# cshizhe/VLN-HAMT

Hardware: AMD Instinct MI355X
Metric: panorama-steps/sec, R2R proxy pretrain (36x768 views, 80-tok instr) (higher is better)
Workload: dtype bf16; 1 GPU; R2R 6-proxy-task pretrain step (fwd+bwd+clip+AdamW, dropout 0.1), fixed ViT features, R2R-canon model 174.8M params; per_gpu_batch=64, global_batch=64, txt_len=80, hist_len=5, views=36, task_mix=mlm:sap:sar:sprel:mrc:itm=5:1:1:1:2:2, parallelism=dp1, launch=hipGraph replay, dead_code_elimination=True

## Files before the change

### include/hamt.h

```cpp
#ifndef HAMT_H
#define HAMT_H

#include <stddef.h>
#include <stdint.h>

#ifdef __cplusplus
extern "C" {
#endif

#define HAMT_ABI_VERSION 2

typedef enum { HAMT_OK = 0, HAMT_ERR_ARG = -1, HAMT_ERR_UNSUPPORTED = -2, HAMT_ERR_LAUNCH = -3 } hamt_status;
typedef enum { HAMT_F32 = 0, HAMT_BF16 = 1,
               HAMT_U8G = 2,
               HAMT_F16 = 3 } hamt_dtype;
typedef enum { HAMT_PREC_BF16 = 0, HAMT_PREC_F32 = 1 } hamt_prec;

int hamt_version(void);
int hamt_last_error(char* buf, size_t n);
int hamt_last_kernel(char* buf, size_t n);
enum { HAMT_WS_GEMM_SPLITK = 0, HAMT_WS_COLSUM = 1, HAMT_WS_SUMSQ = 2, HAMT_WS_LN_BWD = 3, HAMT_WS_WGRAD_TABLE = 4, HAMT_WS_LNRED_TABLE = 5, HAMT_WS_VIS_EMBED_BWD = 6,
       HAMT_WS_EMBED_BWD = 7 ,
       HAMT_WS_OBJ_EMBED_BWD = 8, HAMT_WS_IMAGE_PREP = 9  };
size_t hamt_workspace_bytes(int op, const int* shape, int nshape);
// ... 113 lines not shown
typedef struct {
  const float *w_ang, *b_ang, *w_pos, *b_pos;
  const float *gamma_img, *beta_img, *gamma_ang, *beta_ang, *gamma_pos, *beta_pos;
  const float *tt, *nav, *gamma_out, *beta_out;
} hamt_obj_embed_params;
typedef struct {
  float *dw_ang, *db_ang, *dw_pos, *db_pos;
  float *dgamma_img, *dbeta_img, *dgamma_ang, *dbeta_ang, *dgamma_pos, *dbeta_pos;
  float *dtt, *dnav, *dgamma_out, *dbeta_out;
} hamt_obj_embed_grads;
int hamt_obj_embed_fwd(const hamt_obj_embed_desc* d, const hamt_obj_embed_params* p, const void* x1, const float* ang, const float* pos,
                       float* y, float* stats, const uint64_t* rng, void* stream);
int hamt_obj_embed_bwd(const hamt_obj_embed_desc* d, const hamt_obj_embed_params* p, const hamt_obj_embed_grads* g, const float* dy,
                       const void* x1, const float* ang, const float* pos, const float* stats, float* dx, void* dx16, float* ws,
                       const uint64_t* rng, void* stream);

typedef struct {
  int M, H;
  float eps, p_pre, p_post;
  uint32_t call_id;
  int Mpad16;
  int io16;
} hamt_ln_desc;
#define HAMT_LN_X_BF16 1
#define HAMT_LN_Z_BF16 2
#define HAMT_LN_X_F16 4
#define HAMT_LN_Z_F16 8
int hamt_ln_fwd(const hamt_ln_desc* d, const void* x, const float* residual, const float* gamma,
                const float* beta, void* z, float* y, void* y16, float* mean, float* rstd,
                const uint64_t* rng, void* stream);
int hamt_ln_bwd(const hamt_ln_desc* d, const float* dy, const void* z, const float* mean,
                const float* rstd, const float* gamma, float* dz, float* dx, void* dx16, float* dgamma,
                float* dbeta, float* dxsum, float* ws, const uint64_t* rng, void* stream);
int hamt_ln_bwd_add(const hamt_ln_desc* d, const float* dy, const void* z, const float* mean, const float* rstd,
                    const float* gamma, const float* add, float* dz, float* dgamma, float* dbeta, float* ws,
                    void* stream);
int hamt_ln_bwd_reduce(int M, int H, const float* ws, float* dgamma, float* dbeta, float* dxsum, void* stream);
typedef struct {
  const float* ws;
  float* dgamma;
  float* dbeta;
  float* dxsum;
  int M, H;
  int atomic;
} hamt_ln_reduce_desc;
#define HAMT_LNRED_TABLE_ENTRY 48
int hamt_ln_bwd_reduce_grouped(int n, const hamt_ln_reduce_desc* descs, void* table, size_t table_bytes, void* stream);

int hamt_gather_rows(int R, int W, const float* src, int ld_src, const int64_t* idx, const float* base,
                     int ld_base, float* out, int ld_out, int col0, void* stream);
int hamt_scatter_add_rows(int R, int W, const float* src, int ld_src, int col0, const int64_t* idx,
                          float* dst, int ld_dst, void* stream);
int hamt_scatter_add_rows_ordered(int R, int W, const float* src, int ld_src, int col0, const int64_t* idx,
                                  float* dst, int ld_dst, int T, int* ws, void* stream);
int hamt_scatter_add_rows_small(int R, int W, const float* src, int ld_src, int col0, const int64_t* idx, int T, float* dst,
                                float* ws, void* stream);

int hamt_embed_sum_fwd(int B, int L, int H, const int64_t* ids, const float* word, const float* pos,
                       const float* type_row, float* z, void* stream);
int hamt_embed_sum_bwd(int B, int L, int H, int V, const int64_t* ids, const float* dz, float* dword,
                       float* dpos, float* dtype_row, float* ws, size_t ws_bytes, void* stream);

int hamt_mean_mid_fwd(int B, int S, int H, const float* x, float* y, void* stream);
int hamt_mean_mid_bwd(int B, int S, int H, const float* dy, float* dx, void* stream);
int hamt_mul_bcast_fwd(int B, int S, int H, const float* a, const float* c, int ldc_rows, float* y, void* stream);
int hamt_mul_bcast_bwd(int B, int S, int H, const float* a, const float* c, int ldc_rows, const float* dy,
// ... 179 lines not shown
```

### vln_hamt_amd/_lib.py

```python
from __future__ import annotations

import ctypes as C
import os

_HERE = os.path.dirname(os.path.abspath(__file__))
LIB_PATH = os.path.join(_HERE, "libhamt_hip.so")

HAMT_F32, HAMT_BF16, HAMT_U8G, HAMT_F16 = 0, 1, 2, 3
PREC_BF16, PREC_F32 = 0, 1
EPI_BIAS, EPI_GELU, EPI_RELU, EPI_ACCUM, EPI_MUL_DGELU, EPI_MUL_DRELU, EPI_SAVE_PRE = 1, 2, 4, 8, 16, 32, 64
EPI_GELU_GRAD, EPI_MUL_AUX, EPI_ADD_AUX, EPI_DROPOUT = 128, 256, 512, 1024
SUMSQ_SPARSE = 2
OPT_ADAMW, OPT_ADAM, OPT_RMSPROP, OPT_SGD = 0, 1, 2, 3

vp, i32, u32, f32, sz = C.c_void_p, C.c_int, C.c_uint32, C.c_float, C.c_size_t


class GemmDesc(C.Structure):
    _fields_ = [("M", i32), ("N", i32), ("K", i32), ("lda", i32), ("ldb", i32), ("ldc", i32), ("ldaux", i32),
                ("a_kmajor", i32), ("b_kmajor", i32), ("dtype_a", i32), ("dtype_b", i32), ("dtype_c", i32),
                ("dtype_aux", i32), ("prec", i32), ("epilogue", i32), ("alpha", f32), ("ka_rows", i32), ("kb_rows", i32),
                ("p_drop", f32), ("call_id", u32), ("rng", C.c_void_p)]


# ... 67 lines not shown
                ("ldx", i32), ("ldw", i32), ("accum_dw", i32), ("accum_db", i32), ("ss", vp), ("K_valid", i32),
                ("wire_scale", f32), ("dy2", vp), ("x2", vp), ("K2", i32), ("ldy2", i32), ("ldx2", i32), ("K2_valid", i32)]


SIGNATURES = {
    "hamt_version": [],
    "hamt_last_error": [C.c_char_p, sz],
    "hamt_last_kernel": [C.c_char_p, sz],
    "hamt_workspace_bytes": [i32, C.POINTER(i32), i32],
    "hamt_gemm": [C.POINTER(GemmDesc), vp, vp, vp, vp, vp, vp],
    "hamt_gemm_ksplit": [C.POINTER(GemmDesc)],
    "hamt_gemm_ws": [C.POINTER(GemmDesc), vp, vp, vp, vp, vp, vp, sz, vp],
    "hamt_gemm_plan": [C.POINTER(GemmDesc), sz, C.c_char_p, sz],
    "hamt_cast_pad_bf16": [i32, i32, i32, i32, vp, i32, vp, i32, vp],
    "hamt_cast_pad_bf16_dropout": [i32, i32, i32, vp, i32, vp, i32, f32, u32, vp, vp],
    "hamt_cast_transpose": [i32, i32, vp, i32, i32, vp, i32, i32, vp],
    "hamt_wgrad_grouped": [i32, C.POINTER(WgradDesc), vp, sz, vp],
    "hamt_wgrad_grouped_ex": [i32, C.POINTER(WgradDesc), vp, sz, i32, vp],
    "hamt_smallk_wgrad": [i32, i32, i32, vp, i32, vp, i32, vp, i32, vp, vp],
    "hamt_colsum": [i32, i32, vp, i32, i32, vp, i32, vp, vp],
    "hamt_attn_small_fwd": [C.POINTER(AttnDesc), vp, vp, vp, vp, vp, vp, vp, vp],
    "hamt_attn_small_bwd": [C.POINTER(AttnDesc), vp, vp, vp, vp, vp, vp, vp, vp, vp, vp, vp, vp, vp],
    "hamt_attn_cls_fwd": [C.POINTER(AttnDesc), vp, vp, vp, vp, vp],
    "hamt_attn_varlen_fwd": [C.POINTER(AttnDesc), vp, vp, vp, vp, vp, vp, vp, vp],
    "hamt_attn_varlen_bwd": [C.POINTER(AttnDesc), vp, vp, vp, vp, vp, vp, vp, vp, vp, vp, vp, vp],
    "hamt_attn_varlen_cross_fwd": [C.POINTER(AttnDesc), vp, vp, vp, vp, vp, C.c_int, vp, vp, vp, vp, vp, vp],
    "hamt_attn_varlen_cross_bwd": [C.POINTER(AttnDesc), vp, vp, vp, vp, vp, C.c_int, vp, vp, vp, vp, vp, vp, vp, vp, vp, vp],
    "hamt_vis_embed_fwd": [C.POINTER(VisEmbedDesc)] + [vp] * 12,
    "hamt_vis_embed_bwd": [C.POINTER(VisEmbedDesc)] + [vp] * 18,
    "hamt_obj_embed_fwd": [C.POINTER(ObjEmbedDesc), C.POINTER(ObjEmbedParams)] + [vp] * 7,
    "hamt_obj_embed_bwd": [C.POINTER(ObjEmbedDesc), C.POINTER(ObjEmbedParams), C.POINTER(ObjEmbedGrads)] + [vp] * 10,
    "hamt_ln_fwd": [C.POINTER(LnDesc), vp, vp, vp, vp, vp, vp, vp, vp, vp, vp, vp],
    "hamt_ln_bwd": [C.POINTER(LnDesc), vp, vp, vp, vp, vp, vp, vp, vp, vp, vp, vp, vp, vp, vp],
    "hamt_ln_bwd_add": [C.POINTER(LnDesc), vp, vp, vp, vp, vp, vp, vp, vp, vp, vp, vp],
    "hamt_ln_bwd_reduce": [i32, i32, vp, vp, vp, vp, vp],
    "hamt_ln_bwd_reduce_grouped": [i32, vp, vp, sz, vp],
    "hamt_gather_rows": [i32, i32, vp, i32, vp, vp, i32, vp, i32, i32, vp],
    "hamt_scatter_add_rows": [i32, i32, vp, i32, i32, vp, vp, i32, vp],
    "hamt_scatter_add_rows_small": [i32, i32, vp, i32, i32, vp, i32, vp, vp, vp],
    "hamt_scatter_add_rows_ordered": [i32, i32, vp, i32, i32, vp, vp, i32, i32, vp, vp],
    "hamt_embed_sum_fwd": [i32, i32, i32, vp, vp, vp, vp, vp, vp],
    "hamt_embed_sum_bwd": [i32, i32, i32, i32, vp, vp, vp, vp, vp, vp, sz, vp],
    "hamt_mean_mid_fwd": [i32, i32, i32, vp, vp, vp],
    "hamt_mean_mid_bwd": [i32, i32, i32, vp, vp, vp],
    "hamt_mul_bcast_fwd": [i32, i32, i32, vp, vp, i32, vp, vp],
    "hamt_mul_bcast_bwd": [i32, i32, i32, vp, vp, i32, vp, vp, vp, vp],
    "hamt_sum_rows": [i32, i32, i32, vp, i32, vp, vp, vp],
    "hamt_patchify": [i32, i32, i32, i32, i32, vp, vp, i32, i32, i32, vp],
    "hamt_image_prep": [C.POINTER(ImagePrepDesc), vp, vp, vp, vp, vp, vp, sz, vp],
    "hamt_image_resample_taps": [i32, i32, i32, i32, i32, vp, vp, vp, i32],
    "hamt_image_resample": [C.POINTER(ImageResampleDesc), vp, vp, vp, vp, vp, vp, vp],
    "hamt_add3": [sz, vp, vp, vp, vp, vp],
    "hamt_dropout": [sz, vp, vp, f32, u32, vp, vp],
    "hamt_cast_f32_bf16": [sz, vp, vp, vp],
    "hamt_unpack_padded": [vp, vp, i32, i32, i32, i32, vp, vp],
    "hamt_seq_masks": [vp, i32, i32, i32, vp, vp, vp],
    "hamt_wire_pack_bf16": [C.c_size_t, vp, vp, f32, vp],
    "hamt_wire_unpack_bf16": [C.c_size_t, vp, vp, vp],
    "hamt_fill_where_zero": [sz, vp, vp, f32, vp],
    "hamt_act_bwd": [sz, vp, vp, i32, vp, vp],
    "hamt_ce_fwd": [i32, i32, vp, i32, vp, vp, vp, vp],
    "hamt_ce_bwd": [i32, i32, vp, i32, vp, vp, vp, vp, i32, vp],
    "hamt_mse_fwd": [sz, vp, vp, vp, vp],
    "hamt_mse_bwd": [sz, vp, vp, vp, vp, vp],
    "hamt_kl_fwd": [i32, i32, vp, i32, vp, i32, vp, vp, vp],
    "hamt_kl_bwd": [i32, i32, vp, i32, vp, i32, vp, vp, vp, i32, vp],
# ... 48 lines not shown
        raise HamtError(f"{LIB_PATH} is missing: build it with `python vln_hamt_amd/csrc/build.py` "
                        "(there is no CPU/PyTorch fallback for the HAMT kernels)")
    import torch
    lib = C.CDLL(LIB_PATH)
    for name, args in SIGNATURES.items():
        fn = getattr(lib, name)
        fn.argtypes = args
        fn.restype = sz if name == "hamt_workspace_bytes" else i32
    if lib.hamt_version() != 2:
        raise HamtError("libhamt_hip.so ABI version mismatch")
    _lib = lib
    return lib


def last_error() -> str:
    buf = C.create_string_buffer(512)
    load().hamt_last_error(buf, 512)
    return buf.value.decode(errors="replace")


def last_kernel() -> str:
    buf = C.create_string_buffer(160)
    load().hamt_last_kernel(buf, 160)
    return buf.value.decode(errors="replace")


def gemm_plan(desc: GemmDesc, ws_bytes=None):
    buf = C.create_string_buffer(160)
    ks = load().hamt_gemm_plan(C.byref(desc), sz(-1).value if ws_bytes is None else ws_bytes, buf, 160)
    check(min(ks, 0), "hamt_gemm_plan")
    return ks, buf.value.decode(errors="replace")


def workspace_bytes(op: int, *shape) -> int:
    arr = (i32 * max(1, len(shape)))(*shape)
    return int(load().hamt_workspace_bytes(op, arr, len(shape)))


WS_GEMM_SPLITK, WS_COLSUM, WS_SUMSQ, WS_LN_BWD, WS_WGRAD_TABLE, WS_LNRED_TABLE, WS_VIS_EMBED_BWD, WS_EMBED_BWD, WS_OBJ_EMBED_BWD = range(9)
WS_IMAGE_PREP = 9


def check(rc: int, name: str):
    if rc != 0:
        raise HamtError(f"{name} failed (status {rc}): {last_error()}")
```

### vln_hamt_amd/csrc/ln_row.h

```cpp
#pragma once
#include "common.h"

enum { LN_F32 = 0, LN_BF16 = 1, LN_F16 = 4 };
constexpr int LN_ANGLE_K = 4;

__device__ __forceinline__ float4 zero4() { return make_float4(0.f, 0.f, 0.f, 0.f); }
__device__ __forceinline__ float4 load_row4(const void* xv, size_t o, int fmt) {
  float4 a;
  if (fmt & LN_F16) {
    const uint2 u = *(const uint2*)((const bf16_t*)xv + o);
    unpack_h2(u.x, a.x, a.y); unpack_h2(u.y, a.z, a.w);
  } else if (fmt & LN_BF16) {
    const uint2 u = *(const uint2*)((const bf16_t*)xv + o);
    a = make_float4(__uint_as_float(u.x << 16), __uint_as_float(u.x & 0xffff0000u), __uint_as_float(u.y << 16), __uint_as_float(u.y & 0xffff0000u));
  } else a = *(const float4*)((const float*)xv + o);
  return a;
}
__device__ __forceinline__ void store_bf4(bf16_t* img, size_t o, const float4 r) { *(uint2*)(img + o) = make_uint2(pack_bf2(r.x, r.y), pack_bf2(r.z, r.w)); }
__device__ __forceinline__ void zero_pad_rows(bf16_t* img, int H, int first, int Mpad16, int step, int lane) {
  for (int row = first; row < Mpad16; row += step)
    for (int c = lane * 4; c < H; c += 256) *(uint2*)(img + (size_t)row * H + c) = make_uint2(0u, 0u);
}

__device__ __forceinline__ float sum4(const float4 v) { return v.x + v.y + v.z + v.w; }
__device__ __forceinline__ float dot4(const float4 a, const float4 b) { return a.x * b.x + a.y * b.y + a.z * b.z + a.w * b.w; }
__device__ __forceinline__ float4 mul4(const float4 a, const float4 b) { return make_float4(a.x * b.x, a.y * b.y, a.z * b.z, a.w * b.w); }
__device__ __forceinline__ float4 scale4(const float4 a, float s) { return make_float4(a.x * s, a.y * s, a.z * s, a.w * s); }
__device__ __forceinline__ void acc4(float4& t, const float4 a) { t.x += a.x; t.y += a.y; t.z += a.z; t.w += a.w; }
__device__ __forceinline__ void fmacc4(float4& t, const float4 a, const float4 b) { t.x += a.x * b.x; t.y += a.y * b.y; t.z += a.z * b.z; t.w += a.w * b.w; }
__device__ __forceinline__ void fmacc4(float4& t, const float4 a, float s) { t.x += a.x * s; t.y += a.y * s; t.z += a.z * s; t.w += a.w * s; }
__device__ __forceinline__ float sqdev4(const float4 v, float m) {
  const float e0 = v.x - m, e1 = v.y - m, e2 = v.z - m, e3 = v.w - m;
  return e0 * e0 + e1 * e1 + e2 * e2 + e3 * e3;
}
__device__ __forceinline__ float4 norm4(const float4 v, float m, float r) {
  return make_float4((v.x - m) * r, (v.y - m) * r, (v.z - m) * r, (v.w - m) * r);
}
__device__ __forceinline__ float4 affine4(const float4 n, const float4 g, const float4 b) {
  return make_float4(n.x * g.x + b.x, n.y * g.y + b.y, n.z * g.z + b.z, n.w * g.w + b.w);
}
__device__ __forceinline__ float4 ln_dx4(const float4 u, const float4 n, float cu, float eu, float r) {
  return make_float4(r * (u.x - cu - n.x * eu), r * (u.y - cu - n.y * eu), r * (u.z - cu - n.z * eu), r * (u.w - cu - n.w * eu));
}
__device__ __forceinline__ float4 keep4(RngKey k, int row, int c, float p, float inv_keep) {
  float f[4];
  drop_scale4(k, hamt_mix32((uint32_t)row ^ k.k0), (uint32_t)(c >> 2), p, inv_keep, f);
  return make_float4(f[0], f[1], f[2], f[3]);
}

__device__ __forceinline__ float4 angle_proj4(const float* __restrict__ W, const float* __restrict__ b, int c, const float4 x) {
  const float4* w = (const float4*)(W + (size_t)c * LN_ANGLE_K);
  const float4 w0 = w[0], w1 = w[1], w2 = w[2], w3 = w[3];
  const float4 bb = *(const float4*)(b + c);
  float4 a;
  a.x = bb.x + x.x * w0.x + x.y * w0.y + x.z * w0.z + x.w * w0.w;
  a.y = bb.y + x.x * w1.x + x.y * w1.y + x.z * w1.z + x.w * w1.w;
  a.z = bb.z + x.x * w2.x + x.y * w2.y + x.z * w2.z + x.w * w2.w;
  a.w = bb.w + x.x * w3.x + x.y * w3.y + x.z * w3.z + x.w * w3.w;
  return a;
}

template <int NV, int NWV>
__device__ __forceinline__ void block_partial(const float4 (&t)[NV], float* __restrict__ ws, size_t vec, int H) {
  __shared__ float4 red[NWV][NV * 64];
  const int lane = threadIdx.x & 63, w = threadIdx.x >> 6;
#pragma unroll
  for (int i = 0; i < NV; ++i) red[w][i * 64 + lane] = t[i];
  __syncthreads();
  for (int e = threadIdx.x; e < NV * 64; e += 64 * NWV) {
    const int c = e * 4;
    if (c < H) {
      float4 s = red[0][e];
#pragma unroll
      for (int k = 1; k < NWV; ++k) acc4(s, red[k][e]);
      *(float4*)(ws + vec * H + c) = s;
// ... 39 lines not shown
```

### vln_hamt_amd/csrc/norm.hip

```cpp
#include "ln_row.h"

namespace {

constexpr uint32_t POST_SALT = 0x5bd1e995u;

static_assert(HAMT_LN_X_BF16 == LN_BF16 && HAMT_LN_X_F16 == LN_F16 && HAMT_LN_Z_BF16 == 2 * LN_BF16 && HAMT_LN_Z_F16 == 2 * LN_F16, "io16 layout");
__device__ __forceinline__ int ln_xfmt(int io16) { return io16 & (LN_BF16 | LN_F16); }
__device__ __forceinline__ int ln_zfmt(int io16) { return (io16 >> 1) & (LN_BF16 | LN_F16); }

template <int NV>
__global__ __launch_bounds__(256) void ln_fwd_kernel(hamt_ln_desc d, const void* __restrict__ xv,
                                                     const float* __restrict__ res, const float* __restrict__ gamma,
                                                     const float* __restrict__ beta, void* __restrict__ zv,
                                                     float* __restrict__ y, bf16_t* __restrict__ y16,
                                                     float* __restrict__ mean_o, float* __restrict__ rstd_o,
                                                     const uint64_t* __restrict__ rng) {
  const int lane = threadIdx.x & 63, w = threadIdx.x >> 6;
  const int row = blockIdx.x * 4 + w;
  const int H = d.H;
  if (row >= d.M) {
    if (y16) zero_pad_rows(y16, H, row, d.Mpad16, gridDim.x * 4, lane);
    return;
  }
  const RngKey kpre = rng_key(rng, d.call_id), kpost = rng_key(rng, d.call_id ^ POST_SALT);
  const float ik_pre = d.p_pre > 0.f ? 1.0f / (1.0f - d.p_pre) : 1.0f, ik_post = d.p_post > 0.f ? 1.0f / (1.0f - d.p_post) : 1.0f;
  const int xfmt = ln_xfmt(d.io16);
  float4 v[NV];
  float sum = 0.f;
#pragma unroll
  for (int i = 0; i < NV; ++i) {
    const int c = (i * 64 + lane) * 4;
    if (c < H) {
      const size_t o = (size_t)row * H + c;
      float4 a = load_row4(xv, o, xfmt);
      if (d.p_pre > 0.f) a = mul4(a, keep4(kpre, row, c, d.p_pre, ik_pre));
      if (res) acc4(a, *(const float4*)(res + o));
      v[i] = a;
      sum += sum4(a);
    } else v[i] = zero4();
  }
  const float mean = wave_sum(sum) / (float)H;
  float sq = 0.f;
#pragma unroll
  for (int i = 0; i < NV; ++i)
    if ((i * 64 + lane) * 4 < H) sq += sqdev4(v[i], mean);
  const float rstd = rsqrtf(wave_sum(sq) / (float)H + d.eps);
#pragma unroll
  for (int i = 0; i < NV; ++i) {
    const int c = (i * 64 + lane) * 4;
    if (c < H) {
      const size_t o = (size_t)row * H + c;
      if (zv) {
        if (d.io16 & HAMT_LN_Z_F16) *(uint2*)((bf16_t*)zv + o) = make_uint2(pack_h2(v[i].x, v[i].y), pack_h2(v[i].z, v[i].w));
        else if (d.io16 & HAMT_LN_Z_BF16) store_bf4((bf16_t*)zv, o, v[i]);
        else *(float4*)((float*)zv + o) = v[i];
      }
      float4 r = affine4(norm4(v[i], mean, rstd), *(const float4*)(gamma + c), *(const float4*)(beta + c));
      if (d.p_post > 0.f) r = mul4(r, keep4(kpost, row, c, d.p_post, ik_post));
      if (y) *(float4*)(y + o) = r;
      if (y16) store_bf4(y16, o, r);
    }
  }
  if (lane == 0) { mean_o[row] = mean; rstd_o[row] = rstd; }
}

template <int NV, int NWV>
__global__ __launch_bounds__(64 * NWV) void ln_bwd_kernel(hamt_ln_desc d, const float* __restrict__ dy,
                                                     const void* __restrict__ zv, const float* __restrict__ mean_i,
                                                     const float* __restrict__ rstd_i, const float* __restrict__ gamma,
                                                     float* __restrict__ dz, float* __restrict__ dx, bf16_t* __restrict__ dx16,
                                                     float* __restrict__ ws, const uint64_t* __restrict__ rng,
                                                     const float* __restrict__ add) {
  const int lane = threadIdx.x & 63, w = threadIdx.x >> 6;
  const int H = d.H;
  if (dx16 && blockIdx.x == 0) zero_pad_rows(dx16, H, d.M + w, d.Mpad16, NWV, lane);
  const RngKey kpre = rng_key(rng, d.call_id), kpost = rng_key(rng, d.call_id ^ POST_SALT);
  const float ik_pre = d.p_pre > 0.f ? 1.0f / (1.0f - d.p_pre) : 1.0f, ik_post = d.p_post > 0.f ? 1.0f / (1.0f - d.p_post) : 1.0f;
  const int zfmt = ln_zfmt(d.io16);
  float4 gam[NV], dg[NV], db[NV], dxs[NV];
#pragma unroll
  for (int i = 0; i < NV; ++i) {
    const int c = (i * 64 + lane) * 4;
    gam[i] = c < H ? *(const float4*)(gamma + c) : zero4();
    dg[i] = zero4(); db[i] = zero4(); dxs[i] = zero4();
  }
  for (int row = blockIdx.x * NWV + w; row < d.M; row += gridDim.x * NWV) {
    const float mean = mean_i[row], rstd = rstd_i[row];
    float4 g[NV], xh[NV];
    float s1 = 0.f, s2 = 0.f;
#pragma unroll
    for (int i = 0; i < NV; ++i) {
      const int c = (i * 64 + lane) * 4;
      if (c < H) {
        const size_t o = (size_t)row * H + c;
        float4 a = *(const float4*)(dy + o);
        if (d.p_post > 0.f) a = mul4(a, keep4(kpost, row, c, d.p_post, ik_post));
        const float4 h = norm4(load_row4(zv, o, zfmt), mean, rstd);
        fmacc4(dg[i], a, h);
        acc4(db[i], a);
        a = mul4(a, gam[i]);
        s1 += a.x + a.y + a.z + a.w;
        s2 += a.x * h.x + a.y * h.y + a.z * h.z + a.w * h.w;
        g[i] = a; xh[i] = h;
      }
    }
    const float c1 = wave_sum(s1) / (float)H, c2 = wave_sum(s2) / (float)H;
#pragma unroll
    for (int i = 0; i < NV; ++i) {
      const int c = (i * 64 + lane) * 4;
      if (c < H) {
        const size_t o = (size_t)row * H + c;
        float4 r = ln_dx4(g[i], xh[i], c1, c2, rstd);
        if (add) {
          const float4 q = *(const float4*)(add + o);
          *(float4*)(dz + o) = make_float4(r.x + q.x, r.y + q.y, r.z + q.z, r.w + q.w);
        } else *(float4*)(dz + o) = r;
        if (d.p_pre > 0.f) r = mul4(r, keep4(kpre, row, c, d.p_pre, ik_pre));
        if (dx) *(float4*)(dx + o) = r;
        if (dx16) store_bf4(dx16, o, r);
        acc4(dxs[i], r);
      }
    }
  }
  __shared__ float4 red[NWV > 4 ? NWV / 2 : 4][3][NV * 64];
#pragma unroll
  for (int half = NWV / 2; half >= 4; half >>= 1) {
    if (w >= half && w < 2 * half) {
#pragma unroll
      for (int i = 0; i < NV; ++i) { red[w - half][0][i * 64 + lane] = dg[i]; red[w - half][1][i * 64 + lane] = db[i]; red[w - half][2][i * 64 + lane] = dxs[i]; }
    }
    __syncthreads();
    if (w < half) {
#pragma unroll
      for (int i = 0; i < NV; ++i) {
        const float4 a = red[w][0][i * 64 + lane], b = red[w][1][i * 64 + lane], c = red[w][2][i * 64 + lane];
        acc4(dg[i], a); acc4(db[i], b); acc4(dxs[i], c);
      }
    }
    __syncthreads();
  }
  if (w < 4) {
#pragma unroll
    for (int i = 0; i < NV; ++i) { red[w][0][i * 64 + lane] = dg[i]; red[w][1][i * 64 + lane] = db[i]; red[w][2][i * 64 + lane] = dxs[i]; }
  }
  __syncthreads();
  if (w < 3) {
#pragma unroll
    for (int i = 0; i < NV; ++i) {
      const int c = (i * 64 + lane) * 4;
      if (c < H) {
        float4 a = red[0][w][i * 64 + lane], b = red[1][w][i * 64 + lane], cc = red[2][w][i * 64 + lane], e = red[3][w][i * 64 + lane];
        *(float4*)(ws + ((size_t)blockIdx.x * 3 + w) * H + c) = make_float4(a.x + b.x + cc.x + e.x, a.y + b.y + cc.y + e.y, a.z + b.z + cc.z + e.z, a.w + b.w + cc.w + e.w);
      }
    }
  }
}

__global__ __launch_bounds__(1024) void ln_bwd_reduce_kernel(int nb, int H, const float* __restrict__ ws, float* __restrict__ dgamma,
                                                             float* __restrict__ dbeta, float* __restrict__ dxsum) {
  const int c = blockIdx.x * 64 + (threadIdx.x & 63), ph = threadIdx.x >> 6;
  const int which = c / H, col = c % H;
  float s = 0.f;
  if (c < 3 * H)
    for (int b = ph; b < nb; b += 16) s += ws[((size_t)b * 3 + which) * H + col];
  __shared__ float red[16][64];
// ... 35 lines not shown
  const int blk = blockIdx.x % bpe;
  if (blk * 64 >= 3 * q.H) return;
  int which, col;
  float4 t;
  if (!ln_reduce4(blk, q.nb, q.H, q.ws, which, col, t)) return;
  float* o = which == 0 ? q.dgamma : (which == 1 ? q.dbeta : q.dxsum);
  if (!o) return;
  if ((q.atomic >> which) & 1) {
    atomicAdd(o + col, t.x); atomicAdd(o + col + 1, t.y); atomicAdd(o + col + 2, t.z); atomicAdd(o + col + 3, t.w);
  } else *(float4*)(o + col) = t;
}

}

extern "C" int hamt_ln_fwd(const hamt_ln_desc* d, const void* x, const float* residual, const float* gamma,
                           const float* beta, void* z, float* y, void* y16, float* mean, float* rstd,
                           const uint64_t* rng, void* stream) {
  HAMT_CHECK_ARG(d && x && gamma && beta && (y || y16) && mean && rstd, "hamt_ln_fwd: null pointer");
  HAMT_CHECK_ARG(d->H % 4 == 0 && d->H >= 4 && d->H <= 1024, "hamt_ln_fwd: H=%d unsupported (need H%%4==0, H<=1024)", d->H);
  HAMT_CHECK_ARG(d->p_pre >= 0.f && d->p_pre < 1.f && d->p_post >= 0.f && d->p_post < 1.f, "hamt_ln_fwd: bad dropout p");
  HAMT_CHECK_ARG((d->io16 & (HAMT_LN_X_BF16 | HAMT_LN_X_F16)) != (HAMT_LN_X_BF16 | HAMT_LN_X_F16) && (d->io16 & (HAMT_LN_Z_BF16 | HAMT_LN_Z_F16)) != (HAMT_LN_Z_BF16 | HAMT_LN_Z_F16),
                 "hamt_ln_fwd: io16 = %d names two formats for one tensor", d->io16);
  if (d->M == 0) return HAMT_OK;
  const int rows = (y16 && d->Mpad16 > d->M) ? d->Mpad16 : d->M;
  dim3 grid((rows + 3) / 4), block(256);
  hipStream_t s = as_stream(stream);
#define LAUNCH(NV) hipLaunchKernelGGL((ln_fwd_kernel<NV>), grid, block, 0, s, *d, x, residual, gamma, beta, z, y, (bf16_t*)y16, mean, rstd, rng)
  LN_ROW_DISPATCH(d->H, LAUNCH)
#undef LAUNCH
  HAMT_CHECK_LAUNCH("hamt_ln_fwd");
  return HAMT_OK;
}

static void ln_bwd_geometry(int M, int* nwv_out, int* nb_out) {
  static const int force_w = getenv("HAMT_LN_BWD_WAVES") ? atoi(getenv("HAMT_LN_BWD_WAVES")) : 0;
  const int nwv = force_w ? force_w : (M >= 2048 ? 16 : (M >= 1024 ? 8 : 4));
  int nb = (M + nwv - 1) / nwv;
  if (nb > 256) nb = 256;
  *nwv_out = nwv;
  *nb_out = nb;
}
static void ln_bwd_reduce_launch(int nb, int H, const float* ws, float* dgamma, float* dbeta, float* dxsum, hipStream_t s) {
  const bool al = H % 64 == 0 && (((uintptr_t)dgamma | (uintptr_t)dbeta | (uintptr_t)dxsum | (uintptr_t)ws) % 16) == 0;
  if (al) hipLaunchKernelGGL(ln_bwd_reduce4_kernel, dim3(3 * H / 64), dim3(256), 0, s, nb, H, ws, dgamma, dbeta, dxsum);
  else hipLaunchKernelGGL(ln_bwd_reduce_kernel, dim3((3 * H + 63) / 64), dim3(1024), 0, s, nb, H, ws, dgamma, dbeta, dxsum);
}

static int ln_bwd_impl(const hamt_ln_desc* d, const float* dy, const void* z, const float* mean,
                       const float* rstd, const float* gamma, float* dz, float* dx, void* dx16, float* dgamma,
                       float* dbeta, float* dxsum, float* ws, const uint64_t* rng, const float* add, void* stream) {
  HAMT_CHECK_ARG(d && dy && z && mean && rstd && gamma && dz && ws, "hamt_ln_bwd: null pointer");
  HAMT_CHECK_ARG(d->H % 4 == 0 && d->H >= 4 && d->H <= 1024, "hamt_ln_bwd: H=%d unsupported", d->H);
  HAMT_CHECK_ARG(!(d->p_pre > 0.f) || dx || dx16, "hamt_ln_bwd: p_pre > 0 needs dx or dx16");
  if (d->M == 0) return HAMT_OK;
  int nwv, nb;
  ln_bwd_geometry(d->M, &nwv, &nb);
  hipStream_t s = as_stream(stream);
  float* dxx = d->p_pre > 0.f ? dx : nullptr;
#define LAUNCH2(NV, W) hipLaunchKernelGGL((ln_bwd_kernel<NV, W>), dim3(nb), dim3(64 * W), 0, s, *d, dy, z, mean, rstd, gamma, dz, dxx, (bf16_t*)dx16, ws, rng, add)
#define LAUNCH(NV) { if (nwv == 16) LAUNCH2(NV, 16); else if (nwv == 8) LAUNCH2(NV, 8); else LAUNCH2(NV, 4); }
  LN_ROW_DISPATCH(d->H, LAUNCH)
#undef LAUNCH
#undef LAUNCH2
  if (dgamma || dbeta || dxsum) ln_bwd_reduce_launch(nb, d->H, ws, dgamma, dbeta, dxsum, s);
  HAMT_CHECK_LAUNCH("hamt_ln_bwd");
  return HAMT_OK;
}

extern "C" int hamt_ln_bwd(const hamt_ln_desc* d, const float* dy, const void* z, const float* mean,
                           const float* rstd, const float* gamma, float* dz, float* dx, void* dx16, float* dgamma,
                           float* dbeta, float* dxsum, float* ws, const uint64_t* rng, void* stream) {
  return ln_bwd_impl(d, dy, z, mean, rstd, gamma, dz, dx, dx16, dgamma, dbeta, dxsum, ws, rng, nullptr, stream);
}

extern "C" int hamt_ln_bwd_add(const hamt_ln_desc* d, const float* dy, const void* z, const float* mean,
                               const float* rstd, const float* gamma, const float* add, float* dz, float* dgamma,
                               float* dbeta, float* ws, void* stream) {
  HAMT_CHECK_ARG(add && d && !(d->p_pre > 0.f) && !(d->p_post > 0.f), "hamt_ln_bwd_add: needs `add`, and no dropout inside the LayerNorm");
  return ln_bwd_impl(d, dy, z, mean, rstd, gamma, dz, nullptr, nullptr, dgamma, dbeta, nullptr, ws, nullptr, add, stream);
}

extern "C" int hamt_ln_bwd_reduce(int M, int H, const float* ws, float* dgamma, float* dbeta, float* dxsum, void* stream) {
  HAMT_CHECK_ARG(ws && M >= 0 && H % 4 == 0 && H >= 4 && H <= 1024, "hamt_ln_bwd_reduce: bad argument");
  if (M == 0 || !(dgamma || dbeta || dxsum)) return HAMT_OK;
  int nwv, nb;
  ln_bwd_geometry(M, &nwv, &nb);
  ln_bwd_reduce_launch(nb, H, ws, dgamma, dbeta, dxsum, as_stream(stream));
  HAMT_CHECK_LAUNCH("hamt_ln_bwd_reduce");
  return HAMT_OK;
}

extern "C" int hamt_ln_bwd_reduce_grouped(int n, const hamt_ln_reduce_desc* descs, void* table, size_t table_bytes, void* stream) {
  HAMT_CHECK_ARG(n >= 0 && (n == 0 || (descs && table)), "hamt_ln_bwd_reduce_grouped: bad argument");
  if (n == 0) return HAMT_OK;
  HAMT_CHECK_ARG((size_t)n * sizeof(LnRedEntry) <= table_bytes, "hamt_ln_bwd_reduce_grouped: table too small (%zu bytes needed)", (size_t)n * sizeof(LnRedEntry));
  hipStream_t s = as_stream(stream);
  LnRedEntry* tab = (LnRedEntry*)table;
  int hmax = 0;
  for (int i = 0; i < n; ++i) {
    const hamt_ln_reduce_desc& d = descs[i];
    HAMT_CHECK_ARG(d.ws && d.M > 0 && d.H % 64 == 0 && d.H <= 1024, "hamt_ln_bwd_reduce_grouped: entry %d: needs ws, M > 0, H %% 64 == 0 (H = %d)", i, d.H);
    HAMT_CHECK_ARG((((uintptr_t)d.ws | (uintptr_t)d.dgamma | (uintptr_t)d.dbeta | (uintptr_t)d.dxsum) % 16) == 0, "hamt_ln_bwd_reduce_grouped: entry %d: pointers must be 16-byte aligned", i);
    hmax = d.H > hmax ? d.H : hmax;
  }
  for (int b0 = 0; b0 < n; b0 += LNRED_CHUNK) {
    LnRedChunk ch;
    const int cnt = n - b0 < LNRED_CHUNK ? n - b0 : LNRED_CHUNK;
    for (int i = 0; i < cnt; ++i) {
      const hamt_ln_reduce_desc& d = descs[b0 + i];
      int nwv, nb;
      ln_bwd_geometry(d.M, &nwv, &nb);
      ch.e[i] = LnRedEntry{d.ws, d.dgamma, d.dbeta, d.dxsum, nb, d.H, d.atomic, 0};
    }
    hipLaunchKernelGGL(ln_red_table_write_kernel, dim3(1), dim3(64), 0, s, ch, tab, b0, cnt);
  }
  const int bpe = 3 * hmax / 64;
  hipLaunchKernelGGL(ln_bwd_reduce_grouped_kernel, dim3(n * bpe), dim3(256), 0, s, tab, bpe);
  HAMT_CHECK_LAUNCH("hamt_ln_bwd_reduce_grouped");
  return HAMT_OK;
}
```

Baseline: 6651 panorama-steps/s.

## Restructure LayerNorm backward: contiguous row chunks, shared gamma, fused dy sum entry

Reworks the LayerNorm backward kernel so each block handles a contiguous chunk of rows rather than a grid-strided set. Gamma is staged in shared memory instead of registers, loads are issued up front per row, and the z format is specialized at compile time. A new hamt_ln_bwd_sum entry sums two upstream gradients inside the kernel, and the wave count is capped for wide rows. The aim is lower register pressure and better memory-level parallelism, plus removal of a separate add pass when callers adopt the new entry. The cost is extra shared memory and a barrier, and the reduction order changes slightly.

Result: no change. 6669 panorama-steps/s, median of 6 (+0.3%).

```diff
diff --git a/include/hamt.h b/include/hamt.h
--- a/include/hamt.h
+++ b/include/hamt.h
@@ -169,6 +169,10 @@
 int hamt_ln_bwd(const hamt_ln_desc* d, const float* dy, const void* z, const float* mean,
                 const float* rstd, const float* gamma, float* dz, float* dx, void* dx16, float* dgamma,
                 float* dbeta, float* dxsum, float* ws, const uint64_t* rng, void* stream);
+int hamt_ln_bwd_sum(const hamt_ln_desc* d, const float* dy, const float* dy2, const void* z, const float* mean,
+                    const float* rstd, const float* gamma, float* dz, float* dx, void* dx16, float* dgamma,
+                    float* dbeta, float* dxsum, float* ws, const uint64_t* rng, void* stream);
+int hamt_ln_bwd_plan(int M, int H, int* waves, int* blocks, int* rows);
 int hamt_ln_bwd_add(const hamt_ln_desc* d, const float* dy, const void* z, const float* mean, const float* rstd,
                     const float* gamma, const float* add, float* dz, float* dgamma, float* dbeta, float* ws,
                     void* stream);
diff --git a/vln_hamt_amd/_lib.py b/vln_hamt_amd/_lib.py
--- a/vln_hamt_amd/_lib.py
+++ b/vln_hamt_amd/_lib.py
@@ -123,6 +123,8 @@
     "hamt_obj_embed_bwd": [C.POINTER(ObjEmbedDesc), C.POINTER(ObjEmbedParams), C.POINTER(ObjEmbedGrads)] + [vp] * 10,
     "hamt_ln_fwd": [C.POINTER(LnDesc), vp, vp, vp, vp, vp, vp, vp, vp, vp, vp, vp],
     "hamt_ln_bwd": [C.POINTER(LnDesc), vp, vp, vp, vp, vp, vp, vp, vp, vp, vp, vp, vp, vp, vp],
+    "hamt_ln_bwd_sum": [C.POINTER(LnDesc), vp, vp, vp, vp, vp, vp, vp, vp, vp, vp, vp, vp, vp, vp, vp],
+    "hamt_ln_bwd_plan": [i32, i32, C.POINTER(i32), C.POINTER(i32), C.POINTER(i32)],
     "hamt_ln_bwd_add": [C.POINTER(LnDesc), vp, vp, vp, vp, vp, vp, vp, vp, vp, vp, vp],
     "hamt_ln_bwd_reduce": [i32, i32, vp, vp, vp, vp, vp],
     "hamt_ln_bwd_reduce_grouped": [i32, vp, vp, sz, vp],
@@ -237,6 +239,12 @@
     return ks, buf.value.decode(errors="replace")
 
 
+def ln_bwd_plan(M: int, H: int):
+    w, b, r = i32(), i32(), i32()
+    check(load().hamt_ln_bwd_plan(M, H, C.byref(w), C.byref(b), C.byref(r)), "hamt_ln_bwd_plan")
+    return w.value, b.value, r.value
+
+
 def workspace_bytes(op: int, *shape) -> int:
     arr = (i32 * max(1, len(shape)))(*shape)
     return int(load().hamt_workspace_bytes(op, arr, len(shape)))
diff --git a/vln_hamt_amd/csrc/ln_bwd_plan.h b/vln_hamt_amd/csrc/ln_bwd_plan.h
--- /dev/null
+++ b/vln_hamt_amd/csrc/ln_bwd_plan.h
@@ -0,0 +1,23 @@
+#pragma once
+
+constexpr int LN_BWD_MAX_BLOCKS = 256;
+
+struct LnBwdTuning {
+  int waves;
+};
+
+struct LnBwdPlan {
+  int waves;
+  int blocks;
+  int rows;
+};
+
+static inline LnBwdPlan ln_bwd_plan(int M, int H, LnBwdTuning t = LnBwdTuning{0}) {
+  LnBwdPlan p;
+  p.waves = (t.waves == 4 || t.waves == 8 || t.waves == 16) ? t.waves : (M >= 2048 ? 16 : (M >= 1024 ? 8 : 4));
+  if (H > 768 && p.waves > 8) p.waves = 8;
+  p.rows = 1;
+  const int nb = (M + p.waves - 1) / p.waves;
+  p.blocks = nb > LN_BWD_MAX_BLOCKS ? LN_BWD_MAX_BLOCKS : (nb < 1 ? 1 : nb);
+  return p;
+}
diff --git a/vln_hamt_amd/csrc/ln_row.h b/vln_hamt_amd/csrc/ln_row.h
--- a/vln_hamt_amd/csrc/ln_row.h
+++ b/vln_hamt_amd/csrc/ln_row.h
@@ -14,6 +14,23 @@
     const uint2 u = *(const uint2*)((const bf16_t*)xv + o);
     a = make_float4(__uint_as_float(u.x << 16), __uint_as_float(u.x & 0xffff0000u), __uint_as_float(u.y << 16), __uint_as_float(u.y & 0xffff0000u));
   } else a = *(const float4*)((const float*)xv + o);
+  return a;
+}
+__device__ __forceinline__ float4 load_raw4(const void* xv, size_t o, int fmt) {
+  if (fmt & (LN_F16 | LN_BF16)) {
+    const uint2 u = *(const uint2*)((const bf16_t*)xv + o);
+    return make_float4(__uint_as_float(u.x), __uint_as_float(u.y), 0.f, 0.f);
+  }
+  return *(const float4*)((const float*)xv + o);
+}
+__device__ __forceinline__ float4 raw_row4(const float4 r, int fmt) {
+  const uint32_t ux = __float_as_uint(r.x), uy = __float_as_uint(r.y);
+  float4 a = r;
+  if (fmt & LN_F16) {
+    unpack_h2(ux, a.x, a.y); unpack_h2(uy, a.z, a.w);
+  } else if (fmt & LN_BF16) {
+    a = make_float4(__uint_as_float(ux << 16), __uint_as_float(ux & 0xffff0000u), __uint_as_float(uy << 16), __uint_as_float(uy & 0xffff0000u));
+  }
   return a;
 }
 __device__ __forceinline__ void store_bf4(bf16_t* img, size_t o, const float4 r) { *(uint2*)(img + o) = make_uint2(pack_bf2(r.x, r.y), pack_bf2(r.z, r.w)); }
@@ -41,6 +58,20 @@
 }
 __device__ __forceinline__ float4 ln_dx4(const float4 u, const float4 n, float cu, float eu, float r) {
   return make_float4(r * (u.x - cu - n.x * eu), r * (u.y - cu - n.y * eu), r * (u.z - cu - n.z * eu), r * (u.w - cu - n.w * eu));
+}
+__device__ __forceinline__ void ln_bwd_acc4(const float4 a, const float4 h, const float4 gm, float4& dg, float4& db, float4& u, float& s1, float& s2) {
+#pragma clang fp contract(off)
+  dg.x = __builtin_fmaf(a.x, h.x, dg.x); dg.y = __builtin_fmaf(a.y, h.y, dg.y); dg.z = __builtin_fmaf(a.z, h.z, dg.z); dg.w = __builtin_fmaf(a.w, h.w, dg.w);
+  db.x = a.x + db.x; db.y = a.y + db.y; db.z = a.z + db.z; db.w = a.w + db.w;
+  u = make_float4(a.x * gm.x, a.y * gm.y, a.z * gm.z, a.w * gm.w);
+  const float hy = h.y * u.y, hz = h.z * u.z, hw = h.w * u.w;
+  s1 = s1 + ((__builtin_fmaf(a.y, gm.y, u.x) + u.z) + u.w);
+  s2 = s2 + ((__builtin_fmaf(h.x, u.x, hy) + hz) + hw);
+}
+__device__ __forceinline__ float4 ln_bwd_dx4(const float4 u, const float4 n, float cu, float eu, float r) {
+#pragma clang fp contract(off)
+  return make_float4(r * __builtin_fmaf(-eu, n.x, u.x - cu), r * __builtin_fmaf(-eu, n.y, u.y - cu), r * __builtin_fmaf(-eu, n.z, u.z - cu),
+                     r * __builtin_fmaf(-eu, n.w, u.w - cu));
 }
 __device__ __forceinline__ float4 keep4(RngKey k, int row, int c, float p, float inv_keep) {
   float f[4];
diff --git a/vln_hamt_amd/csrc/norm.hip b/vln_hamt_amd/csrc/norm.hip
--- a/vln_hamt_amd/csrc/norm.hip
+++ b/vln_hamt_amd/csrc/norm.hip
@@ -1,4 +1,5 @@
 #include "ln_row.h"
+#include "ln_bwd_plan.h"
 
 namespace {
 
@@ -64,73 +65,111 @@
   if (lane == 0) { mean_o[row] = mean; rstd_o[row] = rstd; }
 }
 
+template <int NV>
+__device__ __forceinline__ bool ln_live(int i, int c, int H) { return i < NV - 1 || c < H; }
+
+template <int NV, int NWV, int ZFMT>
+__device__ __forceinline__ void ln_bwd_rows(const hamt_ln_desc& d, const int first, const int n, const int w, const int lane,
+                                            const float* __restrict__ dy, const float* __restrict__ dy2, const void* __restrict__ zv,
+                                            const float* __restrict__ mean_i, const float* __restrict__ rstd_i, float* __restrict__ dz,
+                                            float* __restrict__ dx, bf16_t* __restrict__ dx16, const float* __restrict__ add,
+                                            const RngKey kpre, const RngKey kpost, const float ik_pre, const float ik_post,
+                                            const float4* gam, float4 (&dg)[NV], float4 (&db)[NV], float4 (&dxs)[NV]) {
+  const int H = d.H;
+  for (int row = first + w; row < first + n; row += NWV) {
+    float4 g[NV], xh[NV];
+    const float mean = mean_i[row], rstd = rstd_i[row];
+#pragma unroll
+    for (int i = 0; i < NV; ++i) {
+      const int c = (i * 64 + lane) * 4;
+      g[i] = *(const float4*)(dy + (size_t)row * H + (ln_live<NV>(i, c, H) ? c : 0));
+    }
+    if (dy2) {
+      float4 q[NV];
+#pragma unroll
+      for (int i = 0; i < NV; ++i) {
+        const int c = (i * 64 + lane) * 4;
+        q[i] = *(const float4*)(dy2 + (size_t)row * H + (ln_live<NV>(i, c, H) ? c : 0));
+      }
+#pragma unroll
+      for (int i = 0; i < NV; ++i) acc4(g[i], q[i]);
+    }
+#pragma unroll
+    for (int i = 0; i < NV; ++i) {
+      const int c = (i * 64 + lane) * 4;
+      xh[i] = load_raw4(zv, (size_t)row * H + (ln_live<NV>(i, c, H) ? c : 0), ZFMT);
+    }
+    float s1 = 0.f, s2 = 0.f;
+#pragma unroll
+    for (int i = 0; i < NV; ++i) {
+      const int c = (i * 64 + lane) * 4;
+      if (ln_live<NV>(i, c, H)) {
+        float4 a = g[i];
+        if (d.p_post > 0.f) a = mul4(a, keep4(kpost, row, c, d.p_post, ik_post));
+        const float4 h = norm4(raw_row4(xh[i], ZFMT), mean, rstd);
+        ln_bwd_acc4(a, h, gam[i * 64 + lane], dg[i], db[i], g[i], s1, s2);
+        xh[i] = h;
+      }
+    }
+    const float c1 = wave_sum(s1) / (float)H, c2 = wave_sum(s2) / (float)H;
+#pragma unroll
+    for (int i = 0; i < NV; ++i) {
+      const int c = (i * 64 + lane) * 4;
+      if (ln_live<NV>(i, c, H)) {
+        const size_t o = (size_t)row * H + c;
+        float4 t = ln_bwd_dx4(g[i], xh[i], c1, c2, rstd);
+        if (add) {
+          const float4 q = *(const float4*)(add + o);
+          *(float4*)(dz + o) = make_float4(t.x + q.x, t.y + q.y, t.z + q.z, t.w + q.w);
+        } else *(float4*)(dz + o) = t;
+        if (d.p_pre > 0.f) t = mul4(t, keep4(kpre, row, c, d.p_pre, ik_pre));
+        if (dx) *(float4*)(dx + o) = t;
+        if (dx16) store_bf4(dx16, o, t);
+        acc4(dxs[i], t);
+      }
+    }
+  }
+}
+
 template <int NV, int NWV>
 __global__ __launch_bounds__(64 * NWV) void ln_bwd_kernel(hamt_ln_desc d, const float* __restrict__ dy,
                                                      const void* __restrict__ zv, const float* __restrict__ mean_i,
                                                      const float* __restrict__ rstd_i, const float* __restrict__ gamma,
                                                      float* __restrict__ dz, float* __restrict__ dx, bf16_t* __restrict__ dx16,
                                                      float* __restrict__ ws, const uint64_t* __restrict__ rng,
-                                                     const float* __restrict__ add) {
-  const int lane = threadIdx.x & 63, w = threadIdx.x >> 6;
+                                                     const float* __restrict__ add, const float* __restrict__ dy2) {
+  const int lane = threadIdx.x & 63, w = __builtin_amdgcn_readfirstlane(threadIdx.x >> 6);
   const int H = d.H;
   if (dx16 && blockIdx.x == 0) zero_pad_rows(dx16, H, d.M + w, d.Mpad16, NWV, lane);
   const RngKey kpre = rng_key(rng, d.call_id), kpost = rng_key(rng, d.call_id ^ POST_SALT);
   const float ik_pre = d.p_pre > 0.f ? 1.0f / (1.0f - d.p_pre) : 1.0f, ik_post = d.p_post > 0.f ? 1.0f / (1.0f - d.p_post) : 1.0f;
   const int zfmt = ln_zfmt(d.io16);
-  float4 gam[NV], dg[NV], db[NV], dxs[NV];
+  __shared__ float4 gam[NV * 64];
+  float4 dg[NV], db[NV], dxs[NV];
 #pragma unroll
   for (int i = 0; i < NV; ++i) {
     const int c = (i * 64 + lane) * 4;
-    gam[i] = c < H ? *(const float4*)(gamma + c) : zero4();
+    if (w == 0) gam[i * 64 + lane] = c < H ? *(const float4*)(gamma + c) : zero4();
     dg[i] = zero4(); db[i] = zero4(); dxs[i] = zero4();
   }
-  for (int row = blockIdx.x * NWV + w; row < d.M; row += gridDim.x * NWV) {
-    const float mean = mean_i[row], rstd = rstd_i[row];
-    float4 g[NV], xh[NV];
-    float s1 = 0.f, s2 = 0.f;
-#pragma unroll
-    for (int i = 0; i < NV; ++i) {
-      const int c = (i * 64 + lane) * 4;
-      if (c < H) {
-        const size_t o = (size_t)row * H + c;
-        float4 a = *(const float4*)(dy + o);
-        if (d.p_post > 0.f) a = mul4(a, keep4(kpost, row, c, d.p_post, ik_post));
-        const float4 h = norm4(load_row4(zv, o, zfmt), mean, rstd);
-        fmacc4(dg[i], a, h);
-        acc4(db[i], a);
-        a = mul4(a, gam[i]);
-        s1 += a.x + a.y + a.z + a.w;
-        s2 += a.x * h.x + a.y * h.y + a.z * h.z + a.w * h.w;
-        g[i] = a; xh[i] = h;
-      }
-    }
-    const float c1 = wave_sum(s1) / (float)H, c2 = wave_sum(s2) / (float)H;
-#pragma unroll
-    for (int i = 0; i < NV; ++i) {
-      const int c = (i * 64 + lane) * 4;
-      if (c < H) {
-        const size_t o = (size_t)row * H + c;
-        float4 r = ln_dx4(g[i], xh[i], c1, c2, rstd);
-        if (add) {
-          const float4 q = *(const float4*)(add + o);
-          *(float4*)(dz + o) = make_float4(r.x + q.x, r.y + q.y, r.z + q.z, r.w + q.w);
-        } else *(float4*)(dz + o) = r;
-        if (d.p_pre > 0.f) r = mul4(r, keep4(kpre, row, c, d.p_pre, ik_pre));
-        if (dx) *(float4*)(dx + o) = r;
-        if (dx16) store_bf4(dx16, o, r);
-        acc4(dxs[i], r);
-      }
-    }
-  }
+  __syncthreads();
+  const int q = d.M / (int)gridDim.x, rem = d.M % (int)gridDim.x, b = blockIdx.x;
+  const int first = b * q + (b < rem ? b : rem), n = q + (b < rem ? 1 : 0);
+#define LN_BWD_ROWS(F) ln_bwd_rows<NV, NWV, F>(d, first, n, w, lane, dy, dy2, zv, mean_i, rstd_i, dz, dx, dx16, add, kpre, kpost, ik_pre, ik_post, gam, dg, db, dxs)
+  if (zfmt & LN_F16) LN_BWD_ROWS(LN_F16);
+  else if (zfmt & LN_BF16) LN_BWD_ROWS(LN_BF16);
+  else LN_BWD_ROWS(LN_F32);
+#undef LN_BWD_ROWS
   __shared__ float4 red[NWV > 4 ? NWV / 2 : 4][3][NV * 64];
 #pragma unroll
-  for (int half = NWV / 2; half >= 4; half >>= 1) {
-    if (w >= half && w < 2 * half) {
+  for (int n = NWV; n > 4; n /= 2) {
+    const int half = n / 2;
+    if (w >= half && w < n) {
 #pragma unroll
       for (int i = 0; i < NV; ++i) { red[w - half][0][i * 64 + lane] = dg[i]; red[w - half][1][i * 64 + lane] = db[i]; red[w - half][2][i * 64 + lane] = dxs[i]; }
     }
     __syncthreads();
-    if (w < half) {
+    if (w < n - half) {
 #pragma unroll
       for (int i = 0; i < NV; ++i) {
         const float4 a = red[w][0][i * 64 + lane], b = red[w][1][i * 64 + lane], c = red[w][2][i * 64 + lane];
@@ -232,13 +271,20 @@
   return HAMT_OK;
 }
 
-static void ln_bwd_geometry(int M, int* nwv_out, int* nb_out) {
+static LnBwdTuning ln_bwd_tuning() {
   static const int force_w = getenv("HAMT_LN_BWD_WAVES") ? atoi(getenv("HAMT_LN_BWD_WAVES")) : 0;
-  const int nwv = force_w ? force_w : (M >= 2048 ? 16 : (M >= 1024 ? 8 : 4));
-  int nb = (M + nwv - 1) / nwv;
-  if (nb > 256) nb = 256;
-  *nwv_out = nwv;
-  *nb_out = nb;
+  return LnBwdTuning{force_w};
+}
+template <int NV>
+static void ln_bwd_launch(const LnBwdPlan& p, hipStream_t s, const hamt_ln_desc& d, const float* dy, const void* z, const float* mean, const float* rstd,
+                          const float* gamma, float* dz, float* dx, bf16_t* dx16, float* ws, const uint64_t* rng, const float* add, const float* dy2) {
+#define LAUNCH3(W) hipLaunchKernelGGL((ln_bwd_kernel<NV, W>), dim3(p.blocks), dim3(64 * W), 0, s, d, dy, z, mean, rstd, gamma, dz, dx, dx16, ws, rng, add, dy2)
+  if constexpr (NV < 4) {
+    if (p.waves == 16) { LAUNCH3(16); return; }
+  }
+  if (p.waves == 8) LAUNCH3(8);
+  else LAUNCH3(4);
+#undef LAUNCH3
 }
 static void ln_bwd_reduce_launch(int nb, int H, const float* ws, float* dgamma, float* dbeta, float* dxsum, hipStream_t s) {
   const bool al = H % 64 == 0 && (((uintptr_t)dgamma | (uintptr_t)dbeta | (uintptr_t)dxsum | (uintptr_t)ws) % 16) == 0;
@@ -246,23 +292,20 @@
   else hipLaunchKernelGGL(ln_bwd_reduce_kernel, dim3((3 * H + 63) / 64), dim3(1024), 0, s, nb, H, ws, dgamma, dbeta, dxsum);
 }
 
-static int ln_bwd_impl(const hamt_ln_desc* d, const float* dy, const void* z, const float* mean,
+static int ln_bwd_impl(const hamt_ln_desc* d, const float* dy, const float* dy2, const void* z, const float* mean,
                        const float* rstd, const float* gamma, float* dz, float* dx, void* dx16, float* dgamma,
                        float* dbeta, float* dxsum, float* ws, const uint64_t* rng, const float* add, void* stream) {
   HAMT_CHECK_ARG(d && dy && z && mean && rstd && gamma && dz && ws, "hamt_ln_bwd: null pointer");
   HAMT_CHECK_ARG(d->H % 4 == 0 && d->H >= 4 && d->H <= 1024, "hamt_ln_bwd: H=%d unsupported", d->H);
   HAMT_CHECK_ARG(!(d->p_pre > 0.f) || dx || dx16, "hamt_ln_bwd: p_pre > 0 needs dx or dx16");
   if (d->M == 0) return HAMT_OK;
-  int nwv, nb;
-  ln_bwd_geometry(d->M, &nwv, &nb);
+  const LnBwdPlan p = ln_bwd_plan(d->M, d->H, ln_bwd_tuning());
   hipStream_t s = as_stream(stream);
   float* dxx = d->p_pre > 0.f ? dx : nullptr;
-#define LAUNCH2(NV, W) hipLaunchKernelGGL((ln_bwd_kernel<NV, W>), dim3(nb), dim3(64 * W), 0, s, *d, dy, z, mean, rstd, gamma, dz, dxx, (bf16_t*)dx16, ws, rng, add)
-#define LAUNCH(NV) { if (nwv == 16) LAUNCH2(NV, 16); else if (nwv == 8) LAUNCH2(NV, 8); else LAUNCH2(NV, 4); }
+#define LAUNCH(NV) ln_bwd_launch<NV>(p, s, *d, dy, z, mean, rstd, gamma, dz, dxx, (bf16_t*)dx16, ws, rng, add, dy2)
   LN_ROW_DISPATCH(d->H, LAUNCH)
 #undef LAUNCH
-#undef LAUNCH2
-  if (dgamma || dbeta || dxsum) ln_bwd_reduce_launch(nb, d->H, ws, dgamma, dbeta, dxsum, s);
+  if (dgamma || dbeta || dxsum) ln_bwd_reduce_launch(p.blocks, d->H, ws, dgamma, dbeta, dxsum, s);
   HAMT_CHECK_LAUNCH("hamt_ln_bwd");
   return HAMT_OK;
 }
@@ -270,22 +313,35 @@
 extern "C" int hamt_ln_bwd(const hamt_ln_desc* d, const float* dy, const void* z, const float* mean,
                            const float* rstd, const float* gamma, float* dz, float* dx, void* dx16, float* dgamma,
                            float* dbeta, float* dxsum, float* ws, const uint64_t* rng, void* stream) {
-  return ln_bwd_impl(d, dy, z, mean, rstd, gamma, dz, dx, dx16, dgamma, dbeta, dxsum, ws, rng, nullptr, stream);
+  return ln_bwd_impl(d, dy, nullptr, z, mean, rstd, gamma, dz, dx, dx16, dgamma, dbeta, dxsum, ws, rng, nullptr, stream);
+}
+
+extern "C" int hamt_ln_bwd_sum(const hamt_ln_desc* d, const float* dy, const float* dy2, const void* z, const float* mean,
+                               const float* rstd, const float* gamma, float* dz, float* dx, void* dx16, float* dgamma,
+                               float* dbeta, float* dxsum, float* ws, const uint64_t* rng, void* stream) {
+  return ln_bwd_impl(d, dy, dy2, z, mean, rstd, gamma, dz, dx, dx16, dgamma, dbeta, dxsum, ws, rng, nullptr, stream);
 }
 
 extern "C" int hamt_ln_bwd_add(const hamt_ln_desc* d, const float* dy, const void* z, const float* mean,
                                const float* rstd, const float* gamma, const float* add, float* dz, float* dgamma,
                                float* dbeta, float* ws, void* stream) {
   HAMT_CHECK_ARG(add && d && !(d->p_pre > 0.f) && !(d->p_post > 0.f), "hamt_ln_bwd_add: needs `add`, and no dropout inside the LayerNorm");
-  return ln_bwd_impl(d, dy, z, mean, rstd, gamma, dz, nullptr, nullptr, dgamma, dbeta, nullptr, ws, nullptr, add, stream);
+  return ln_bwd_impl(d, dy, nullptr, z, mean, rstd, gamma, dz, nullptr, nullptr, dgamma, dbeta, nullptr, ws, nullptr, add, stream);
+}
+
+extern "C" int hamt_ln_bwd_plan(int M, int H, int* waves, int* blocks, int* rows) {
+  HAMT_CHECK_ARG(M >= 1 && H % 4 == 0 && H >= 4 && H <= 1024, "hamt_ln_bwd_plan: bad argument (M = %d, H = %d)", M, H);
+  const LnBwdPlan p = ln_bwd_plan(M, H, ln_bwd_tuning());
+  if (waves) *waves = p.waves;
+  if (blocks) *blocks = p.blocks;
+  if (rows) *rows = p.rows;
+  return HAMT_OK;
 }
 
 extern "C" int hamt_ln_bwd_reduce(int M, int H, const float* ws, float* dgamma, float* dbeta, float* dxsum, void* stream) {
   HAMT_CHECK_ARG(ws && M >= 0 && H % 4 == 0 && H >= 4 && H <= 1024, "hamt_ln_bwd_reduce: bad argument");
   if (M == 0 || !(dgamma || dbeta || dxsum)) return HAMT_OK;
-  int nwv, nb;
-  ln_bwd_geometry(M, &nwv, &nb);
-  ln_bwd_reduce_launch(nb, H, ws, dgamma, dbeta, dxsum, as_stream(stream));
+  ln_bwd_reduce_launch(ln_bwd_plan(M, H, ln_bwd_tuning()).blocks, H, ws, dgamma, dbeta, dxsum, as_stream(stream));
   HAMT_CHECK_LAUNCH("hamt_ln_bwd_reduce");
   return HAMT_OK;
 }
@@ -308,9 +364,7 @@
     const int cnt = n - b0 < LNRED_CHUNK ? n - b0 : LNRED_CHUNK;
     for (int i = 0; i < cnt; ++i) {
       const hamt_ln_reduce_desc& d = descs[b0 + i];
-      int nwv, nb;
-      ln_bwd_geometry(d.M, &nwv, &nb);
-      ch.e[i] = LnRedEntry{d.ws, d.dgamma, d.dbeta, d.dxsum, nb, d.H, d.atomic, 0};
+      ch.e[i] = LnRedEntry{d.ws, d.dgamma, d.dbeta, d.dxsum, ln_bwd_plan(d.M, d.H, ln_bwd_tuning()).blocks, d.H, d.atomic, 0};
     }
     hipLaunchKernelGGL(ln_red_table_write_kernel, dim3(1), dim3(64), 0, s, ch, tab, b0, cnt);
   }
```
